# ChangUk/RecommenderSystems

Measured on AMD Instinct MI355X. Metric: RWR seeds/sec + achieved HBM GB/s on 100M-edge bipartite graph, 1/2/4/8 GPUs, higher is better.
Workload: dtype f64

## Files before the change

include/rwr.h:

```cpp
#ifndef RWR_H
#define RWR_H

#include <stdint.h>

#ifdef __cplusplus
extern "C" {
#endif

#define RWR_VERSION_STRING "0.4.0"

enum {
    RWR_OK            = 0,
    RWR_E_INVALID     = 1,
    RWR_E_RANGE       = 2,
    RWR_E_NO_DEVICE   = 3,
    RWR_E_HIP         = 4,
    RWR_E_NOMEM       = 5,
    RWR_E_CAPACITY    = 6,
    RWR_E_UNSUPPORTED = 7
};

enum { RWR_NODE_UNDEFINED = 0, RWR_NODE_USER = 1, RWR_NODE_ITEM = 2, RWR_NODE_ETC = 3 };
enum { RWR_EDGE_UNDEFINED = 0, RWR_EDGE_LIKE = 1, RWR_EDGE_FRIENDSHIP = 2, RWR_EDGE_FOLLOW = 3,
       RWR_EDGE_MENTION = 4, RWR_EDGE_AUTHORSHIP = 5, RWR_EDGE_PURCHASE = 6, RWR_EDGE_ETC = 7 };
// ... 17 lines not shown
} rwr_opts;

typedef struct rwr_stats {
    int32_t struct_size;
    int32_t n;
    int64_t nnz_raw;
    int64_t nnz;
    int32_t uniform;
    int32_t tile_seeds;
    int32_t tile_group;
    int32_t mode;
    double  build_ms;
    double  spmm_ms;
    int64_t spmm_launches;
    int64_t spmm_seed_steps;
    double  chain_ms;
    int64_t chain_launches;
    double  rank_ms;
    double  iterate_wall_ms;
    double  total_wall_ms;
    int64_t seeds_done;
    int64_t chain_redo_blocks;
    double  spmm_dense_ms;
    int64_t spmm_dense_launches;
    int64_t spmm_dense_seed_steps;
    int32_t uniform_path;
    int32_t reserved1;
    int64_t frontier_list_launches;
    int64_t rank_fused_groups;
    int64_t rank_fused_fallbacks;
    int64_t rank_pruned_rows;
    double  rank_bound_ms;
    int64_t x_clear_skipped;
} rwr_stats;


const char *rwr_version(void);
int32_t rwr_device_count(void);
const char *rwr_last_error(void);

int32_t rwr_graph_create(int32_t n, const int64_t *node_id, const uint8_t *node_type,
                         const int64_t *rowptr , const int32_t *dst, const uint8_t *etype,
                         const double *w, const rwr_opts *opts , rwr_graph **out);
int32_t rwr_graph_destroy(rwr_graph *g);
int32_t rwr_graph_update_links(rwr_graph *g, int64_t count, const int64_t *link_index,
                               const uint8_t *etype , const double *w );
int32_t rwr_graph_append_links(rwr_graph *g, int64_t count, const int32_t *src, const int32_t *dst,
                               const uint8_t *etype, const double *w,
                               int64_t *new_index_out );
int32_t rwr_graph_append_nodes(rwr_graph *g, int32_t n_new, const int64_t *node_id,
                               const uint8_t *node_type, int64_t count, const int32_t *src,
                               const int32_t *dst, const uint8_t *etype, const double *w,
                               int64_t *new_index_out );
int32_t rwr_graph_size(const rwr_graph *g, int32_t *n, int64_t *nnz_raw, int64_t *nnz_explicit);
int32_t rwr_graph_get_normalized(rwr_graph *g, double *w_out , uint8_t *dangling_out );

int32_t rwr_recommend(rwr_graph *g, int32_t seed, float d, int32_t n_iter, int32_t top_n,
                      int64_t *out_id, double *out_score, int64_t *inout_count);

int32_t rwr_recommend_eval(rwr_graph *g, int32_t seed, float d, int32_t n_iter, const int64_t *test_ids,
                           int64_t n_test, int64_t *n_hits, double *sum_precision, int64_t *list_len);

int32_t rwr_recommend_eval_batch(rwr_graph *g, const int32_t *seeds, int32_t K, float d, int32_t n_iter,
                                 const int64_t *test_ptr, const int64_t *test_ids, int64_t *n_hits,
                                 double *sum_precision, int64_t *list_len);

// ... 59 lines not shown
```

recommendersystems_amd/_lib.py:

```python
from __future__ import annotations

import ctypes as C
import os

_HERE = os.path.dirname(os.path.abspath(__file__))
LIB_PATH = os.path.join(_HERE, "librwr.so")

RWR_OK, RWR_E_INVALID, RWR_E_RANGE, RWR_E_NO_DEVICE, RWR_E_HIP, RWR_E_NOMEM, RWR_E_CAPACITY, RWR_E_UNSUPPORTED = range(8)
RWR_MODE_EXACT = 0
RWR_RUN_ITERATIONS, RWR_RUN_THRESHOLD, RWR_RUN_DEFAULT_THRESHOLD = 0, 1, 2

EXPORTS = [
    "rwr_version", "rwr_device_count", "rwr_last_error",
    "rwr_graph_create", "rwr_graph_update_links", "rwr_graph_append_links", "rwr_graph_append_nodes", "rwr_graph_destroy", "rwr_graph_size", "rwr_graph_get_normalized",
    "rwr_recommend", "rwr_recommend_eval", "rwr_recommend_eval_batch", "rwr_eval_graphs", "rwr_recommend_batch", "rwr_model_run", "rwr_model_deliver",
    "rwr_model_run_restart", "rwr_model_deliver_restart", "rwr_model_run_batch", "rwr_model_run_restart_batch",
    "rwr_recommend_restart_batch", "rwr_recommend_restart_eval_batch", "rwr_recommend_typed_batch",
    "rwr_part_begin", "rwr_part_step", "rwr_part_local_step", "rwr_part_finish_step", "rwr_part_rank",
    "rwr_get_stats", "rwr_reset_stats",
]


class rwr_opts(C.Structure):
    _fields_ = [("struct_size", C.c_int32), ("device", C.c_int32), ("mode", C.c_int32),
                ("tile_seeds", C.c_int32), ("tile_group", C.c_int32), ("profile", C.c_int32),
                ("workspace_bytes", C.c_int64), ("seed_row_kernel", C.c_int32), ("reserved0", C.c_int32)]


class rwr_graph_desc(C.Structure):
    _fields_ = [("n_nodes", C.c_int32), ("reserved0", C.c_int32), ("node_id", C.POINTER(C.c_int64)),
                ("node_type", C.POINTER(C.c_uint8)), ("rowptr", C.POINTER(C.c_int64)), ("dst", C.POINTER(C.c_int32)),
                ("etype", C.POINTER(C.c_uint8)), ("w", C.POINTER(C.c_double))]


class rwr_stats(C.Structure):
    _fields_ = [("struct_size", C.c_int32), ("n", C.c_int32), ("nnz_raw", C.c_int64), ("nnz", C.c_int64),
                ("uniform", C.c_int32), ("tile_seeds", C.c_int32), ("tile_group", C.c_int32), ("mode", C.c_int32),
                ("build_ms", C.c_double), ("spmm_ms", C.c_double), ("spmm_launches", C.c_int64),
                ("spmm_seed_steps", C.c_int64), ("chain_ms", C.c_double), ("chain_launches", C.c_int64),
                ("rank_ms", C.c_double), ("iterate_wall_ms", C.c_double), ("total_wall_ms", C.c_double),
                ("seeds_done", C.c_int64), ("chain_redo_blocks", C.c_int64),
                ("spmm_dense_ms", C.c_double), ("spmm_dense_launches", C.c_int64), ("spmm_dense_seed_steps", C.c_int64),
                ("uniform_path", C.c_int32), ("reserved1", C.c_int32), ("frontier_list_launches", C.c_int64),
                ("rank_fused_groups", C.c_int64), ("rank_fused_fallbacks", C.c_int64),
                ("rank_pruned_rows", C.c_int64), ("rank_bound_ms", C.c_double), ("x_clear_skipped", C.c_int64)]


class RwrError(RuntimeError):
    def __init__(self, status: int, message: str):
        super().__init__(f"librwr status {status}: {message}")
        self.status = status


_lib = None


def load():
    global _lib
    if _lib is not None:
        return _lib
    if not os.path.exists(LIB_PATH):
        raise ImportError(f"{LIB_PATH} not found: build it with `python -c 'import __graft_entry__ as g; g.build()'` "
                          "(hipcc --offload-arch=gfx950); there is no CPU fallback")
    lib = C.CDLL(LIB_PATH)
    p = C.POINTER
    lib.rwr_version.restype = C.c_char_p
    lib.rwr_last_error.restype = C.c_char_p
    lib.rwr_device_count.restype = C.c_int32
    lib.rwr_graph_create.restype = C.c_int32
    lib.rwr_graph_create.argtypes = [C.c_int32, p(C.c_int64), p(C.c_uint8), p(C.c_int64), p(C.c_int32),
                                     p(C.c_uint8), p(C.c_double), p(rwr_opts), p(C.c_void_p)]
    lib.rwr_graph_update_links.restype = C.c_int32
    lib.rwr_graph_update_links.argtypes = [C.c_void_p, C.c_int64, p(C.c_int64), p(C.c_uint8), p(C.c_double)]
    lib.rwr_graph_append_links.restype = C.c_int32
    lib.rwr_graph_append_links.argtypes = [C.c_void_p, C.c_int64, p(C.c_int32), p(C.c_int32), p(C.c_uint8), p(C.c_double),
                                           p(C.c_int64)]
    lib.rwr_graph_append_nodes.restype = C.c_int32
    lib.rwr_graph_append_nodes.argtypes = [C.c_void_p, C.c_int32, p(C.c_int64), p(C.c_uint8), C.c_int64, p(C.c_int32), p(C.c_int32),
# ... 72 lines not shown
```

recommendersystems_amd/csrc/api.hip:

```cpp
#include <stdarg.h>
#include <algorithm>
#include <cmath>
#include <vector>
#include <string.h>

#include "eval_plan.h"
#include "exclude_plan.h"
#include "handle.h"
#include "rank.h"

namespace rwr {

static thread_local char g_err[512] = "";

void set_error(const char *fmt, ...)
{
    va_list ap;
    va_start(ap, fmt);
    vsnprintf(g_err, sizeof(g_err), fmt, ap);
    va_end(ap);
}

template <class F>
static int32_t bound(const char *who, rwr_graph *g, F &&body)
// ... 602 lines not shown
}

int32_t rwr_part_rank(rwr_graph *g, void *dev_x, int32_t top_n, int64_t *ids, double *scores, int32_t *counts)
{
    g_err[0] = 0;
    if (!g || !dev_x || !ids || !scores || !counts) { set_error("rwr_part_rank: NULL argument"); return RWR_E_INVALID; }
    return bound("rwr_part_rank", g, [&] { return part_rank(g, (double *)dev_x, top_n, ids, scores, counts); });
}

int32_t rwr_get_stats(rwr_graph *g, rwr_stats *out)
{
    if (!g || !out) { set_error("rwr_get_stats: NULL argument"); return RWR_E_INVALID; }
    size_t sz = out->struct_size > 0 ? (size_t)out->struct_size : sizeof(rwr_stats);
    if (sz > sizeof(rwr_stats)) sz = sizeof(rwr_stats);
    rwr_stats s = g->stats;
    s.struct_size = (int32_t)sz;
    memcpy(out, &s, sz);
    return RWR_OK;
}

int32_t rwr_reset_stats(rwr_graph *g)
{
    if (!g) { set_error("rwr_reset_stats: NULL argument"); return RWR_E_INVALID; }
    rwr_stats &s = g->stats;
    s.spmm_ms = s.chain_ms = s.rank_ms = s.iterate_wall_ms = s.total_wall_ms = 0;
    s.spmm_launches = s.spmm_seed_steps = s.chain_launches = s.seeds_done = s.chain_redo_blocks = 0;
    s.spmm_dense_ms = 0;
    s.spmm_dense_launches = s.spmm_dense_seed_steps = 0;
    s.frontier_list_launches = 0;
    s.rank_fused_groups = s.rank_fused_fallbacks = 0;
    s.rank_pruned_rows = 0;
    s.rank_bound_ms = 0;
    s.x_clear_skipped = 0;
    return RWR_OK;
}

}
```

recommendersystems_amd/csrc/engine.h:

```cpp
#pragma once
#include <cstdlib>
#include <new>

#include "cand_plan.h"
#include "common.h"
#include "stage_layout.h"

struct rwr_graph {
    int32_t device = 0;
    int32_t n = 0;
    int64_t nnz_raw = 0;
    int64_t nnz = 0;
    int32_t n_items = 0;
    uint64_t id_key_top = 0;
    int32_t id_key_bits = 64;
    uint64_t id_key_lo = 0;
    int32_t id_key_lo_known = 0;
    int32_t uniform = 0;
    int32_t vf = 0;
    int32_t nonneg = 1;
    int32_t max_in_deg = 0;
    int32_t staged = 0;
    int32_t stage_pending = 0;
    int32_t poisoned = 0;
// ... 29 lines not shown
    rwr::DevBuf<int32_t> tail_rows[TAIL_MAX];
    int32_t tail_n[TAIL_MAX] = {0, 0, 0, 0};
    int32_t tail_depth = 0;
    std::vector<uint8_t> h_tail_flag;
    int32_t tail_state = 0;
    rwr::DevBuf<int32_t> cand_rows[rwr::CAND_CACHE];
    rwr::CandEntry cand_entry[rwr::CAND_CACHE];
    uint64_t cand_calls = 0;

    int32_t sw_state = 0, sw_B = 0, sw_BN = 0, sw_K = 0, sw_nwg = 0, sw_wpg = 0, sw_hub0 = 0;
    int32_t sw_rows = 0;
    int32_t sw_partial = 0;
    rwr::DevBuf<uint32_t> sw_wgblk;
    int64_t sw_words = 0;
    rwr::DevBuf<int32_t> sw_order;
    rwr::DevBuf<uint4> sw_meta;
    rwr::DevBuf<uint2> sw_ent;

    rwr::DevBuf<double> X, Y;
    rwr::DevBuf<int32_t> sm_tab;
    void *sm_pin = nullptr;
    void *sm_stage = nullptr;
    uint8_t *sm_out = nullptr;
    const uint8_t *stage_dev_ext = nullptr;
    rwr::DevBuf<uint8_t> d_stage;
    int32_t sm_pin_count = -1;
    rwr::DevBuf<double> Z0, Z1;
    rwr::DevBuf<int32_t> d_seeds;
    rwr::DevBuf<int32_t> d_slot_k;
    rwr::DevBuf<double> d_part;
    rwr::DevBuf<unsigned int> d_gate;
    rwr::DevBuf<uint32_t> d_nz;
    rwr::DevBuf<int32_t> fl_rows;
    rwr::DevBuf<int64_t> d_evoff;
    rwr::DevBuf<double> d_evterm;
    rwr::DevBuf<double> cs_approx;
    rwr::DevBuf<int32_t> cs_e;
    rwr::DevBuf<long long> cs_d0, cs_d1;
    rwr::DevBuf<double> cs_side;
    rwr::DevBuf<double> cs_mx;
    rwr::DevBuf<int32_t> cs_lnk;
    rwr::DevBuf<int32_t> cs_lnk0;
    rwr::DevBuf<double> cs_diff;
    rwr::DevBuf<double> cs_sums;
    rwr::DevBuf<int32_t> mb_row;
    rwr::DevBuf<unsigned long long> cs_redo;
    rwr::DevBuf<uint64_t> keys, keys_alt;
    rwr::DevBuf<uint32_t> vals, vals_alt;
    rwr::DevBuf<uint8_t> sort_temp;
    rwr::DevBuf<uint8_t> fused_ws;
    rwr::DevBuf<uint8_t> bound_ws;
    int32_t bound_first = -1, bound_lo = 0, bound_hi = 0;
    rwr::DevBuf<int64_t> d_out_id;
    rwr::DevBuf<double> d_out_score;
    rwr::DevBuf<int32_t> d_counts;

    int32_t part_lo = 0, part_hi = 0, part_G = 0, part_K = 0;
    int32_t part_steps = 0;
    double part_c1 = 0;
    std::vector<int32_t> part_seeds;

    hipStream_t stream = nullptr, stream2 = nullptr;
    hipStream_t stream3 = nullptr;
    hipEvent_t ev_h0 = nullptr, ev_h1 = nullptr;
    hipEvent_t ev_fork = nullptr, ev_join = nullptr;
    hipEvent_t ev_a = nullptr, ev_b = nullptr, ev_c = nullptr, ev_d = nullptr;
// ... 152 lines not shown
```

recommendersystems_amd/csrc/iterate.h:

```cpp
#pragma once
#include "column_ends.h"
#include "engine.h"
#include "rank.h"
#include "step_plan.h"

#include <new>
#include <optional>

namespace rwr {

struct RowScore {
    int32_t row, pad;
    double score;
};
struct SelSink {
    const double *tau = nullptr;
    int32_t *cursor = nullptr;
    RowScore *cand = nullptr;
    int32_t cap = 0, stride = 0;
    int32_t *overflow = nullptr;
    const int32_t *list = nullptr, *list_cnt = nullptr;
    int64_t list_stride = 0;
};

struct SpmmArgs {
    const double *X = nullptr;
    double *Y = nullptr;
    const int32_t *seeds = nullptr;
    double c1 = 0.0;
    bool skip_seed_row = false;
    const uint32_t *nz_in = nullptr;
    uint32_t *nz_out = nullptr;
    const uint32_t *act = nullptr;
    const double *Zin = nullptr;
    double *Zout = nullptr;
    bool hub_scan = false;
    RowSource rows{};
    int32_t row_first = 0, row_count = -1;
    const SelSink *sel = nullptr;
};
void launch_spmm(rwr_graph *g, int G, int tg, const SpmmArgs &a, hipStream_t s);
void launch_init_seeds(rwr_graph *g, int G, int tg, double *X, const int32_t *seeds, uint32_t *nz, double *Z, double c1,
                       hipStream_t s);
void launch_make_z(int64_t elems, int G, const double *X, double *Z, const double *w_src, double c1, hipStream_t s);
void launch_make_z_nz(rwr_graph *g, int32_t lo, int32_t hi, int G, const double *X, double *Zs, double c1, uint32_t *nz,
                      hipStream_t s);
void launch_mark_active(rwr_graph *g, int G, int tg, const uint32_t *nz, uint32_t *act, const int32_t *seeds, int32_t *fl_rows,
                        int32_t *fl_cnt, hipStream_t s);

struct Profile {
    const bool on;
    std::vector<hipEvent_t> pool, spmm, chain, rank, iter, bound;
    size_t used = 0;
    std::vector<uint8_t> dense;
    explicit Profile(const rwr_graph *g) : on(g->opts.profile != 0) {}
    ~Profile() { for (auto e : pool) (void)hipEventDestroy(e); }
    int32_t record(hipEvent_t &e, hipStream_t s);
    int32_t end(std::vector<hipEvent_t> &stage, hipEvent_t a, hipStream_t s);
    void reset() { spmm.clear(); chain.clear(); rank.clear(); iter.clear(); bound.clear(); dense.clear(); used = 0; }
    int32_t fold(rwr_graph *g);
};

struct GroupIter {
    rwr_graph *g;
    int G, tg;
    const int32_t *d_seeds;
    const int64_t *d_evoff;
    double c1;
    double *X, *Y;
    double *Zc = nullptr, *Zn = nullptr;
    uint32_t *nz_cur = nullptr, *nz_oth = nullptr;
    PlanConfig cfg;
// ... 68 lines not shown
```

recommendersystems_amd/csrc/iterate.hip:

```cpp
#include "iterate.h"
#include "spmm_chunk.h"

#include <climits>
#include <cstdlib>
#include <type_traits>

namespace rwr {

template <int G, bool VF>
__global__ __launch_bounds__(256) void k_spmm(int32_t n, const int64_t *__restrict__ in_ptr,
                                              const int32_t *__restrict__ in_src,
                                              const double *__restrict__ in_w,
                                              const int32_t *__restrict__ row_order, int32_t nrows,
                                              const double *__restrict__ X, double *__restrict__ Y,
                                              const int32_t *__restrict__ seeds, double c1, int skip_seed_row,
                                              const double *__restrict__ w_src, double *__restrict__ Zout)
{
    constexpr int RPW = WAVE / G;
    constexpr int U = 4;
    const int tile = blockIdx.y;
    const size_t toff = (size_t)tile * (size_t)n * G;
    X += toff;
    Y += toff;
    if (VF && Zout) Zout += toff;
// ... 16 lines not shown
            int32_t idx[U];
            double wv[U], xv[U];
#pragma unroll
            for (int u = 0; u < U; ++u) idx[u] = in_src[p + u];
#pragma unroll
            for (int u = 0; u < U; ++u) wv[u] = VF ? 0.0 : in_w[p + u];
#pragma unroll
            for (int u = 0; u < U; ++u) xv[u] = X[(size_t)idx[u] * G + k];
#pragma unroll
            for (int u = 0; u < U; ++u) {
                if (VF) {
                    acc += xv[u];
                } else {
                    double rw = c1 * xv[u];
                    acc += rw * wv[u];
                }
            }
        }
        for (; p < e; ++p) {
            if (VF) {
                acc += X[(size_t)in_src[p] * G + k];
            } else {
                double rw = c1 * X[(size_t)in_src[p] * G + k];
                acc += rw * in_w[p];
            }
        }
        if (j >= 0 && j != my_seed) {
            Y[(size_t)j * G + k] = acc;
            if (VF && Zout) { const double rw = c1 * acc; Zout[(size_t)j * G + k] = rw * w_src[j]; }
        }
    }
}

template <int G, int CH, bool CHECK, bool WRITE, bool VF, bool SEL = false>
__device__ __forceinline__ void spmm_chunked_body(int32_t n, const int64_t *__restrict__ in_ptr,
                                                  const int32_t *__restrict__ in_src,
                                                  const double *__restrict__ in_w,
                                                  const int32_t *__restrict__ row_order, int32_t nrows,
                                                  const double *__restrict__ X, double *__restrict__ Y,
                                                  const int32_t *__restrict__ seeds, double c1,
                                                  int skip_seed_row, const uint32_t *__restrict__ nz_in,
                                                  uint32_t *__restrict__ nz_out,
                                                  const uint32_t *__restrict__ act,
                                                  const double *__restrict__ w_src, double *__restrict__ Zout,
                                                  const SelSink sink = SelSink{})
{
    static_assert(G >= 8 && G <= 64, "chunked SpMM needs 8 <= G <= 64");
    static_assert(!SEL || (!CHECK && !WRITE), "the selecting form probes and writes no bitmap");
    constexpr int RPW = WAVE / G;
    constexpr int LW = G <= 32 ? G : VF ? 32 : CH;
    static_assert(LW % CH == 0 && CH <= LW, "an index load is a whole number of gather rounds");
    const int tile = blockIdx.y;
    const size_t toff = (size_t)tile * (size_t)n * G;
    X += toff;
    if (!SEL) Y += toff;
    if (VF && Zout) Zout += toff;
    const size_t nzw = ((size_t)n + 31) / 32;
    if (CHECK) nz_in += (size_t)tile * nzw;
    if (WRITE) nz_out += (size_t)tile * nzw;
    if (CHECK && act) act += (size_t)tile * nzw;
    const int lane = threadIdx.x & (WAVE - 1);
    const int sub = lane / G, k = lane % G;
    const int gbase = (lane - k) << 2;
    const int32_t my_seed = skip_seed_row ? seeds[tile * G + k] : -1;
    bool sel_real = false;
    double sel_tau = 0.0;
    if (SEL) {
        sel_real = seeds[tile * G + k] >= 0;
        sel_tau = sink.tau[tile * G + k];
    }
    const int wpb = blockDim.x / WAVE;
    const int64_t nwaves = (int64_t)gridDim.x * wpb;
    for (int64_t rb = ((int64_t)blockIdx.x * wpb + threadIdx.x / WAVE) * RPW; rb < nrows; rb += nwaves * RPW) {
        const int64_t r = rb + sub;
        int32_t j = -1;
        int64_t p = 0, e = 0;
        if (r < nrows) {
            j = row_order[r];
            p = in_ptr[j];
            e = in_ptr[j + 1];
            if (CHECK && act && !((act[(uint32_t)j >> 5] >> (j & 31)) & 1u)) e = p;
        }
        double acc = 0.0;
        while (__any(p < e)) {
            const int cnt = spmm_next_load(p, e - p, LW);
            int32_t my_idx = 0;
            double my_w = 0.0;
            if (k < cnt) {
                my_idx = in_src[p + k];
                if (!VF) my_w = in_w[p + k];
                if (CHECK) {
                    const uint32_t wd = nz_in[(uint32_t)my_idx >> 5];
                    if (!((wd >> (my_idx & 31)) & 1u)) my_idx |= (int32_t)0x80000000;
                }
            }
            const int wlo = __double2loint(my_w), whi = __double2hiint(my_w);
            unsigned long long um = 0;
            if (CHECK) {
                um = __ballot(k < cnt && my_idx >= 0);
                if (G < 64) {
#pragma unroll
                    for (int sh = G; sh < 64; sh <<= 1) um |= um >> sh;
                    um &= (1ull << (G & 63)) - 1ull;
                }
            }
#pragma unroll G == 64 ? LW / CH : 1
            for (int r0 = 0; r0 < LW; r0 += CH) {
                if (r0 > 0 && !__any(cnt > r0)) break;
                if (CHECK) {
                    unsigned long long rm = (um >> r0) & ((1ull << CH) - 1ull);
                    if (__popcll(rm) <= 4) {
                        while (rm) {
                            const int t = r0 + __builtin_ctzll(rm);
                            rm &= rm - 1;
                            const int idx = __builtin_amdgcn_ds_bpermute(gbase + (t << 2), my_idx);
                            if (VF) {
                                if (t < cnt && idx >= 0) acc += X[(size_t)idx * G + k];
                            } else {
                                const int lo = __builtin_amdgcn_ds_bpermute(gbase + (t << 2), wlo);
                                const int hi = __builtin_amdgcn_ds_bpermute(gbase + (t << 2), whi);
                                if (t < cnt && idx >= 0) {
                                    const double rw = c1 * X[(size_t)idx * G + k];
                                    acc += rw * __hiloint2double(hi, lo);
                                }
// ... 63 lines not shown
}

template <int G, int CH, bool VF>
__global__ __launch_bounds__(256) void k_spmm_select(int32_t n, const int64_t *__restrict__ in_ptr,
                                                     const int32_t *__restrict__ in_src,
                                                     const double *__restrict__ in_w,
                                                     const int32_t *__restrict__ rows, int32_t nrows,
                                                     const double *__restrict__ X, const int32_t *__restrict__ seeds,
                                                     double c1, const SelSink sink)
{
    if (sink.list) {
        rows = sink.list + (size_t)blockIdx.y * (size_t)sink.list_stride;
        nrows = sink.list_cnt[blockIdx.y];
    }
    spmm_chunked_body<G, CH, false, false, VF, true>(n, in_ptr, in_src, in_w, rows, nrows, X, nullptr, seeds, c1, 1, nullptr,
                                                     nullptr, nullptr, nullptr, nullptr, sink);
}

template <int G, int CH, bool VF>
__global__ __launch_bounds__(256) void k_spmm_frontier(int32_t n, const int64_t *__restrict__ in_ptr,
                                                       const int32_t *__restrict__ in_src,
                                                       const double *__restrict__ in_w,
                                                       const int32_t *__restrict__ fl_rows,
                                                       const int32_t *__restrict__ fl_cnt,
                                                       const double *__restrict__ X, double *__restrict__ Y,
                                                       const int32_t *__restrict__ seeds, double c1,
                                                       int skip_seed_row, const uint32_t *__restrict__ nz_in,
                                                       uint32_t *__restrict__ nz_out,
                                                       const double *__restrict__ w_src, double *__restrict__ Zout)
{
    const int tile = blockIdx.y;
    spmm_chunked_body<G, CH, true, true, VF>(n, in_ptr, in_src, in_w, fl_rows + (size_t)tile * (size_t)n, fl_cnt[tile], X, Y,
                                             seeds, c1, skip_seed_row, nz_in, nz_out, nullptr, w_src, Zout);
}

__global__ __launch_bounds__(256) void k_mark_active(int32_t n, const uint32_t *__restrict__ nz, uint32_t *__restrict__ act,
                                                     const int64_t *__restrict__ rowptr, const int32_t *__restrict__ dst,
                                                     const uint8_t *__restrict__ etype, int G, const int32_t *__restrict__ seeds,
                                                     int32_t *__restrict__ fl_rows, int32_t *__restrict__ fl_cnt)
{
    const size_t nzw = ((size_t)n + 31) / 32;
    const int tile = blockIdx.y;
    const int lane = threadIdx.x & (WAVE - 1);
    const size_t wi = (size_t)blockIdx.x * (blockDim.x / WAVE) + threadIdx.x / WAVE;
    uint32_t *a = act + (size_t)tile * nzw;
    int32_t *list = fl_rows ? fl_rows + (size_t)tile * (size_t)n : nullptr;
    if (list && blockIdx.x == 0 && threadIdx.x < (unsigned)G) {
        const int32_t sr = seeds[tile * G + threadIdx.x];
        if (sr >= 0) {
            const uint32_t bit = 1u << (sr & 31);
            if (!(atomicOr(&a[(uint32_t)sr >> 5], bit) & bit)) list[atomicAdd(&fl_cnt[tile], 1)] = sr;
        }
    }
    if (wi >= nzw) return;
    uint32_t w = nz[(size_t)tile * nzw + wi];
    while (w) {
        const int b = __builtin_ctz(w);
        w &= w - 1;
        const int64_t i = (int64_t)wi * 32 + b;
        const int64_t p1 = rowptr[i + 1];
        if (!list) {
            for (int64_t p = rowptr[i] + lane; p < p1; p += WAVE)
                if (etype[p] != RWR_EDGE_UNDEFINED) {
                    const int32_t t = dst[p];
                    atomicOr(&a[(uint32_t)t >> 5], 1u << (t & 31));
                }
// ... 376 lines not shown
    if (j >= lo && j < hi) {
        const double w = w_src[j];
        const size_t at = (size_t)(j - lo) * G;
        for (int k = 0; k < G; ++k) {
            const double xv = X[(size_t)j * G + k];
            const double rw = c1 * xv;
            Zs[at + k] = rw * w;
            any = any || xv != 0.0;
        }
    }
    const unsigned long long m = __ballot(any);
    const int lane = threadIdx.x & (WAVE - 1);
    if (lane == 0 && (uint32_t)m) nz[(uint64_t)j >> 5] = (uint32_t)m;
    if (lane == 32 && (uint32_t)(m >> 32)) nz[(uint64_t)j >> 5] = (uint32_t)(m >> 32);
}


static PlanInput read_plan_knobs()
{
    PlanInput v;
    const char *e;
    if ((e = getenv("RWR_SPMM"))) v.spmm = atoi(e);
    if ((e = RWR_TUNE_ENV("RWR_NZ_ITERS"))) v.nz_iters = atoi(e);
    if ((e = getenv("RWR_ACT_ITERS"))) v.act_iters = atoi(e);
    if ((e = RWR_TUNE_ENV("RWR_ACT_MIN_N"))) v.act_min_n = atol(e);
    if ((e = getenv("RWR_FRONTIER_LIST"))) v.frontier_list = atoi(e);
    if ((e = getenv("RWR_CHAIN"))) v.chain = atoi(e);
    if ((e = RWR_TUNE_ENV("RWR_SCAN_WORK"))) v.scan_work = atof(e);
    if ((e = RWR_TUNE_ENV("RWR_SCAN_SIDE"))) v.scan_side = atoi(e);
    if ((e = RWR_TUNE_ENV("RWR_GATE"))) v.gate = atoi(e);
    if ((e = getenv("RWR_TAIL_ROWS"))) v.tail_rows = atoi(e);
    if ((e = RWR_TUNE_ENV("RWR_CHAIN_SERIAL"))) v.two_streams = atoi(e) == 0;
    if ((e = getenv("RWR_X_CLEAR"))) v.x_clear = atoi(e);
    return v;
}
static const PlanInput &plan_knobs() { static const PlanInput k = read_plan_knobs(); return k; }

template <class F> static void bool_dispatch(F &&f) { f(); }
template <class F, class... B> static void bool_dispatch(F &&f, bool b, B... bs)
{
    bool_dispatch([&](auto... c) { if (b) f(std::true_type{}, c...); else f(std::false_type{}, c...); }, bs...);
}

template <int G>
static void launch_spmm_g(rwr_graph *g, int tg, const SpmmArgs &a, hipStream_t s)
{
    const bool vf = a.Zin != nullptr;
    const double *GS = vf ? a.Zin : a.X;
    const int skip = a.skip_seed_row;
    constexpr int RPW = WAVE / G;
    constexpr int CH = G > 16 ? 16 : G;
    if constexpr (G >= 8) {
        if (a.rows.kind == Rows::Frontier) {
            const int32_t *fl_rows = g->fl_rows.p, *fl_cnt = g->fl_rows.p + (size_t)tg * (size_t)g->n;
            const unsigned want = cdiv((size_t)g->n / 10 + 1, (size_t)RPW * 4);
            const unsigned gx = want < 1u ? 1u : want < 2048u ? want : 2048u;
            bool_dispatch([&](auto v) {
                hipLaunchKernelGGL((k_spmm_frontier<G, CH, decltype(v)::value>), dim3(gx, tg), dim3(256), 0, s, g->n, g->in_ptr.p,
                                   g->in_src.p, g->in_w.p, fl_rows, fl_cnt, GS, a.Y, a.seeds, a.c1, skip, a.nz_in, a.nz_out,
                                   g->w_src.p, a.Zout);
            }, vf);
            return;
        }
    }
    const bool listed = a.rows.kind == Rows::Tail;
    const int32_t *order = listed ? g->tail_rows[a.rows.level].p : g->row_order.p;
    int32_t nrows = listed ? g->tail_n[a.rows.level] : g->n;
    if (listed) {
        const int32_t first = a.row_first < nrows ? a.row_first : nrows;
        order += first;
        nrows = (a.row_count >= 0 && a.row_count < nrows - first) ? a.row_count : nrows - first;
    }
    if (nrows <= 0 && (a.sel || a.row_count >= 0)) return;
    unsigned want = cdiv((size_t)nrows, (size_t)RPW * 4);
    unsigned gx = want < 1u ? 1u : want < 8192u ? want : 8192u;
    if constexpr (G == 1) {
        if (tg == 1 && plan_knobs().spmm != 0) {
            launch_spmv_exact(g, a.X, a.Y, a.seeds, a.c1, skip, a.act, a.nz_out, s, a.Zin, a.Zout, a.hub_scan);
            return;
        }
    }
    if constexpr (G >= 8) {
        if (a.sel) {
            const SelSink sink = *a.sel;
            bool_dispatch([&](auto v) {
                hipLaunchKernelGGL((k_spmm_select<G, CH, decltype(v)::value>), dim3(gx, tg), dim3(256), 0, s, g->n, g->in_ptr.p,
                                   g->in_src.p, g->in_w.p, order, nrows, GS, a.seeds, a.c1, sink);
            }, vf);
            return;
        }
    }
    if constexpr (G >= 8) {
        if (plan_knobs().spmm != 0) {
            bool_dispatch([&](auto chk, auto wr, auto v, auto lst) {
                if constexpr (decltype(chk)::value || !decltype(wr)::value)
                    hipLaunchKernelGGL((k_spmm_chunked<G, CH, decltype(chk)::value, decltype(wr)::value, decltype(v)::value,
                                                       decltype(lst)::value>), dim3(gx, tg), dim3(256), 0, s, g->n, g->in_ptr.p,
                                       g->in_src.p, g->in_w.p, order, nrows, GS, a.Y, a.seeds, a.c1, skip, a.nz_in, a.nz_out,
                                       a.act, g->w_src.p, a.Zout);
            }, a.nz_in != nullptr, a.nz_in && a.nz_out, vf, listed);
            return;
        }
    }
    bool_dispatch([&](auto v) {
        hipLaunchKernelGGL((k_spmm<G, decltype(v)::value>), dim3(gx, tg), dim3(256), 0, s, g->n, g->in_ptr.p, g->in_src.p,
                           g->in_w.p, order, nrows, GS, a.Y, a.seeds, a.c1, skip, g->w_src.p, a.Zout);
    }, vf);
}
void launch_spmm(rwr_graph *g, int G, int tg, const SpmmArgs &a, hipStream_t s)
{
    RWR_DISPATCH_G(G, launch_spmm_g<GG>(g, tg, a, s));
}
void launch_init_seeds(rwr_graph *g, int G, int tg, double *X, const int32_t *seeds, uint32_t *nz, double *Z, double c1,
                       hipStream_t s)
{
    hipLaunchKernelGGL(k_init_seeds, dim3(cdiv((size_t)tg * G, 64)), dim3(64), 0, s, g->n, tg, G, X, seeds, nz, Z, g->w_src.p, c1);
}
void launch_make_z(int64_t elems, int G, const double *X, double *Z, const double *w_src, double c1, hipStream_t s)
{
    hipLaunchKernelGGL(k_make_z, dim3(cdiv((size_t)elems, 256)), dim3(256), 0, s, elems, G, X, Z, w_src, c1);
}
void launch_make_z_nz(rwr_graph *g, int32_t lo, int32_t hi, int G, const double *X, double *Zs, double c1, uint32_t *nz,
                      hipStream_t s)
{
    const int64_t first = (int64_t)lo & ~(int64_t)63;
// ... 67 lines not shown
            *acc += ms;
        }
        return RWR_OK;
    };
    if (on) {
        RWR_TRY(drain(spmm, &g->stats.spmm_dense_ms, true));
        RWR_TRY(drain(spmm, &g->stats.spmm_ms, false));
        RWR_TRY(drain(chain, &g->stats.chain_ms, false));
        RWR_TRY(drain(rank, &g->stats.rank_ms, false));
        RWR_TRY(drain(iter, &g->stats.iterate_wall_ms, false));
        RWR_TRY(drain(bound, &g->stats.rank_bound_ms, false));
    }
    reset();
    return RWR_OK;
}

int32_t GroupIter::init(bool fresh, bool ranks_nonneg, bool ranking_only)
{
    const int32_t n = g->n;
    hipStream_t s = g->stream;
    const size_t elems = (size_t)tg * (size_t)n * G;
    PlanInput in = plan_knobs();
    in.n = n; in.nnz = g->nnz; in.nonneg = g->nonneg; in.big_n = spmv_big_n(); in.seed_row_kernel = g->opts.seed_row_kernel;
    in.scan_self = chain_scan_self_contained(G); in.G = G; in.tg = tg; in.c1 = c1;
    in.fresh = fresh; in.ranks_nonneg = ranks_nonneg; in.ranking_only = ranking_only;
    cfg = plan_config(in);
    if (!fresh && Zc) launch_make_z((int64_t)elems, G, X, Zc, g->w_src.p, c1, s);
    const size_t nzw = ((size_t)n + 31) / 32;
    if (cfg.flist && g->fl_rows.ensure((size_t)tg * (size_t)n + (size_t)tg) != RWR_OK) {
        (void)hipGetLastError();
        cfg.flist = false;
        cfg.clear_x = plan_clear_x(cfg);
    }
    if (fresh && cfg.clear_x) RWR_HIP(hipMemsetAsync(X, 0, elems * sizeof(double), s));
    if (fresh && !cfg.clear_x) g->stats.x_clear_skipped += 1;
    if (fresh && Zc && !cfg.flist) RWR_HIP(hipMemsetAsync(Zc, 0, elems * sizeof(double), s));
    nz_cur = cfg.nz_iters > 0 ? g->d_nz.p : nullptr;
    nz_oth = cfg.nz_iters > 0 ? g->d_nz.p + (size_t)tg * nzw : nullptr;
    if (nz_cur) RWR_HIP(hipMemsetAsync(nz_cur, 0, (size_t)tg * nzw * sizeof(uint32_t), s));
    if (fresh) launch_init_seeds(g, G, tg, X, d_seeds, nz_cur, Zc, c1, s);
    RWR_HIP(hipGetLastError());
    if (cfg.scan) RWR_TRY(chain_scan_prepare(g, G, tg, d_seeds, s));
    if (Zc && G == 1 && tg == 1 && cfg.addends_nonneg) RWR_TRY(sweep_prepare(g));
    if (Zc && cfg.chain_kind == 0 && !cfg.scan) RWR_TRY(ensure_in_w(g));
    return RWR_OK;
}

int32_t GroupIter::step(const StepPlan &p, Profile &prof, int32_t row_first, int32_t row_count)
{
    const int32_t n = g->n;
    hipStream_t s = g->stream;
    const size_t nzw = ((size_t)n + 31) / 32;
    constexpr int GATE_SLOTS = 64;
    const uint32_t *nz_in = p.probe ? nz_cur : nullptr;
    uint32_t *nz_out = p.write_bits ? nz_oth : nullptr;
    if (nz_out) RWR_HIP(hipMemsetAsync(nz_out, 0, (size_t)tg * nzw * sizeof(uint32_t), s));
    uint32_t *act = p.mark ? g->d_nz.p + 2 * (size_t)tg * nzw : nullptr;
    const bool listed = p.rows.kind == Rows::Frontier;
    if (act) {
        int32_t *fl_rows = listed ? g->fl_rows.p : nullptr, *fl_cnt = listed ? fl_rows + (size_t)tg * (size_t)n : nullptr;
        RWR_HIP(hipMemsetAsync(act, 0, (size_t)tg * nzw * sizeof(uint32_t), s));
        if (fl_cnt) RWR_HIP(hipMemsetAsync(fl_cnt, 0, (size_t)tg * sizeof(int32_t), s));
        launch_mark_active(g, G, tg, nz_in, act, d_seeds, fl_rows, fl_cnt, s);
    }
    const uint32_t *nz_terms = p.terms_nz ? nz_in : nullptr;
    double *zout = (Zc && p.form_z) ? Zn : nullptr;
    hipStream_t sc = p.chain_side ? g->stream2 : s;
    unsigned int *gate_it = p.gate ? g->d_gate.p + (it % GATE_SLOTS) : nullptr;
    if (p.chain != Chain::None) {
        if (!p.scan()) RWR_DISPATCH_G(G, launch_seed_terms<GG>(g, tg, X, d_seeds, c1, d_evoff, s, Zc, nz_terms));
        if (gate_it) RWR_HIP(hipMemsetAsync(gate_it, 0, sizeof(unsigned int), s));
        if (p.chain_side) { RWR_HIP(hipEventRecord(g->ev_fork, s)); RWR_HIP(hipStreamWaitEvent(sc, g->ev_fork, 0)); }
        if (p.scan() && !(p.chain_self && Zc)) RWR_DISPATCH_G(G, launch_seed_terms<GG>(g, tg, X, d_seeds, c1, d_evoff, sc, Zc, nz_terms));
        hipEvent_t c0; RWR_TRY(prof.record(c0, sc));
        if (p.scan())
            RWR_TRY(chain_scan_step(g, G, tg, X, Y, d_seeds, d_evoff, c1, nz_out, sc, p.chain_self ? Zc : nullptr,
                                    p.chain_self ? zout : nullptr));
        else
            RWR_DISPATCH_G(G, launch_chain<GG>(g, tg, X, Y, d_seeds, c1, d_evoff, nz_out, gate_it, sc, p.chain, nz_in,
                                                       p.chain_masked));
        RWR_TRY(prof.end(prof.chain, c0, sc));
        if (p.chain_side) RWR_HIP(hipEventRecord(g->ev_join, sc));
    }
    if (gate_it) hipLaunchKernelGGL(k_gate, dim3(1), dim3(1), 0, s, gate_it, (unsigned)(tg < 192 ? tg : 192));
    hipEvent_t a; RWR_TRY(prof.record(a, s));
    SpmmArgs sp;
    sp.X = X, sp.Y = Y, sp.seeds = d_seeds, sp.c1 = c1, sp.skip_seed_row = true;
    sp.nz_in = nz_in, sp.nz_out = nz_out, sp.act = act, sp.Zin = Zc, sp.Zout = zout;
    sp.hub_scan = cfg.addends_nonneg, sp.rows = p.rows;
    sp.row_first = row_first, sp.row_count = row_count;
    launch_spmm(g, G, tg, sp, s);
    RWR_TRY(prof.end(prof.spmm, a, s));
    if (prof.on) prof.dense.push_back(p.dense());
    if (p.dense()) { g->stats.spmm_dense_launches += 1; ++dense_steps; }
    if (p.chain_side) RWR_HIP(hipStreamWaitEvent(s, g->ev_join, 0));
    if (zout && p.seed_z) hipLaunchKernelGGL(k_seed_z, dim3(cdiv((size_t)tg * G, 64)), dim3(64), 0, s, n, tg, G, Y, zout, d_seeds, g->w_src.p, c1);
    RWR_HIP(hipGetLastError());
    { double *t = X; X = Y; Y = t; }
    { double *t = Zc; Zc = Zn; Zn = t; }
    { uint32_t *tz = nz_cur; nz_cur = nz_oth; nz_oth = tz; }
    g->stats.spmm_launches += 1;
    g->stats.chain_launches += p.chain != Chain::None; g->stats.frontier_list_launches += listed;
    ++it;
    return RWR_OK;
}

int32_t GroupIter::redo_rows(const StepPlan &p, Profile &prof, int32_t row_first, int32_t row_count, const SelSink *sel)
{
    hipStream_t s = g->stream;
    hipEvent_t a; RWR_TRY(prof.record(a, s));
    SpmmArgs sp;
    sp.X = Y, sp.Y = X, sp.seeds = d_seeds, sp.c1 = c1, sp.skip_seed_row = true;
    sp.Zin = Zn, sp.Zout = nullptr;
    sp.hub_scan = cfg.addends_nonneg, sp.rows = p.rows;
    sp.row_first = row_first, sp.row_count = row_count, sp.sel = sel;
    launch_spmm(g, G, tg, sp, s);
    RWR_TRY(prof.end(prof.spmm, a, s));
    if (prof.on) prof.dense.push_back(0);
    RWR_HIP(hipGetLastError());
    return RWR_OK;
}

int32_t iterate_group(rwr_graph *g, int G, int tg, const int32_t *d_seeds, const int64_t *d_evoff, const int32_t *h_seeds,
// ... 30 lines not shown
```

recommendersystems_amd/csrc/step_plan.h:

```cpp
#pragma once

#include <cstdint>

namespace rwr {

struct PlanInput {
    int spmm = 1, nz_iters = 4, act_iters = -1, frontier_list = 1, chain = 1, x_clear = 0;
    int64_t act_min_n = 200000; double scan_work = 10000.0;
    int scan_side = 1, gate = 1, tail_rows = 1;
    bool two_streams = true;
    int32_t n = 0, big_n = 2000000;
    int64_t nnz = 0; bool nonneg = true;
    int seed_row_kernel = 0;
    bool scan_self = false;
    int G = 1, tg = 1;
    double c1 = 0.85;
    bool fresh = true;
    bool ranks_nonneg = true;
    bool ranking_only = false;
};

struct PlanConfig {
    int G = 1, tg = 1; bool fresh = true;
    int nz_iters = 0;
    int act_iters = 0;
    bool flist = false;
    bool addends_nonneg = false;
    bool scan = false;
    int chain_kind = 1;
    bool scan_side = false, scan_self = false;
    bool two_streams = true, gate = true;
    bool tails = false; int tail_depth = 0;
    unsigned need = 0;
    bool force_clear = false;
    bool clear_x = true;
};

inline bool plan_clear_x(const PlanConfig &c) { return c.force_clear || !c.flist || c.scan || c.chain_kind == 0; }

inline PlanConfig plan_config(const PlanInput &in)
{
    PlanConfig c;
    c.G = in.G, c.tg = in.tg, c.fresh = in.fresh;
    const bool single = in.G == 1 && in.tg == 1;
    c.nz_iters = (in.G >= 8 && in.spmm != 0 && in.nonneg) ? in.nz_iters : 0;
    c.act_iters = in.act_iters >= 0 ? in.act_iters : ((in.nnz / (in.n > 0 ? in.n : 1)) <= 64 ? 2 : 1);
    if (single && in.act_iters < 0 && c.act_iters == 2 && in.n >= in.big_n) c.act_iters = 3;
    if (single && in.spmm != 0 && in.nonneg) c.nz_iters = c.act_iters;
    if (single && in.act_iters < 0 && in.n < in.act_min_n) c.nz_iters = c.act_iters = 0;
    if (!in.fresh) c.nz_iters = c.act_iters = 0;
    c.flist = in.ranking_only && in.fresh && in.frontier_list != 0 && in.G >= 8 && c.nz_iters >= 2 && c.act_iters >= 1;
    c.chain_kind = in.seed_row_kernel == 1 ? 3 : in.seed_row_kernel == 2 ? 2 : in.seed_row_kernel == 3 ? 0 : in.chain;
    const double per_seed = 0.89 * (double)in.nnz / (double)(in.n > 0 ? in.n : 1) + 6.7;
    c.addends_nonneg = in.c1 >= 0.0 && in.c1 <= 1.0 && in.nonneg && in.ranks_nonneg;
    c.scan = c.addends_nonneg && (c.chain_kind == 2 || (c.chain_kind == 1 && (double)in.tg * in.G * per_seed < in.scan_work));
    c.scan_side = in.scan_side != 0 && single && in.two_streams && in.n >= 100000;
    c.scan_self = in.scan_self, c.two_streams = in.two_streams, c.gate = in.gate != 0;
    c.tails = in.ranking_only && in.tail_rows != 0 && !single;
    c.force_clear = in.x_clear != 0;
    c.clear_x = plan_clear_x(c);
    return c;
}

enum class Rows : uint8_t { All, Frontier, Tail };
struct RowSource { Rows kind = Rows::All; int level = 0; };
enum class Chain : uint8_t { None, Scan, ScanSide, Sparse, Roles, Simple };

struct StepPlan {
    RowSource rows;
    bool probe = false, write_bits = false;
    bool mark = false;
    bool terms_nz = false;
    Chain chain = Chain::None;
    bool chain_masked = false;
    bool chain_side = false, gate = false;
    bool chain_self = false;
    bool form_z = false, seed_z = false;
    bool dense() const { return !probe && rows.kind == Rows::All; }
    bool scan() const { return chain == Chain::Scan || chain == Chain::ScanSide; }
};

inline int last_tail(const PlanConfig &c)
{
    for (int k = 0; c.tails && k < c.tail_depth; ++k)
        if ((c.need >> k) & 1u) return k;
    return c.tails ? c.tail_depth - 1 : -1;
}

inline bool step_lists(const PlanConfig &c, int64_t it, int64_t T)
{
    const int64_t k = T - 1 - it;
    if (!c.flist || T < 0 || it < 0 || k <= 0 || k <= last_tail(c)) return false;
    const bool write_bits = it + 1 < c.nz_iters, mark = it < c.nz_iters && it < c.act_iters;
    return mark && write_bits && (it + 1 < c.act_iters || it == 1);
}

inline StepPlan plan_step(const PlanConfig &c, int64_t it, int64_t T)
{
    StepPlan p;
    const int64_t k = T - 1 - it;
    const bool last = T >= 0 && k == 0, tail = T >= 0 && k <= last_tail(c);
    p.probe = it < c.nz_iters;
    p.write_bits = it + 1 < c.nz_iters;
    p.mark = p.probe && it < c.act_iters;
    p.terms_nz = c.flist && p.probe;
    if (tail)
        p.rows = {Rows::Tail, (int)k};
    else if (step_lists(c, it, T))
        p.rows = {Rows::Frontier, 0};
    if (tail && !((c.need >> k) & 1u)) p.chain = Chain::None;
    else if (c.scan && (!p.mark || c.G == 1)) p.chain = c.scan_side ? Chain::ScanSide : Chain::Scan;
    else if (p.mark) p.chain = Chain::Sparse;
    else p.chain = c.chain_kind == 0 ? Chain::Simple : Chain::Roles;
    p.chain_masked = !c.clear_x && p.chain != Chain::None && p.chain != Chain::Sparse && step_lists(c, it - 1, T);
    const bool fold = p.chain != Chain::None && !p.scan();
    p.chain_side = p.chain == Chain::ScanSide || (fold && c.two_streams);
    p.gate = fold && c.two_streams && c.gate;
    p.chain_self = p.scan() && c.scan_self;
    p.form_z = !last;
    p.seed_z = p.form_z && p.chain != Chain::None && !p.chain_self;
    return p;
}

}
```

Measured before the change: 859.3.

## Precompute per-edge liveness masks to replace random bitmap probes in SpMM

Adds an entry-live path. Each probing step transposes the per-tile nonzero bitmaps into per-node 32-tile words, then expands them into one mask word per CSR entry. The SpMM kernel then reads that mask word instead of gathering a bitmap word indexed by the source node. The goal is to turn scattered bitmap reads into a streamed read aligned with the edge arrays, at the cost of two extra kernels per step that touch every edge and up to several GB of extra workspace. The path is enabled by default only for graphs with at least 100M edges in ranking-only fresh runs.

```diff
diff --git a/include/rwr.h b/include/rwr.h
--- a/include/rwr.h
+++ b/include/rwr.h
@@ -73,6 +73,7 @@
     int64_t rank_pruned_rows;
     double  rank_bound_ms;
     int64_t x_clear_skipped;
+    int64_t entry_live_launches;
 } rwr_stats;
 
 
diff --git a/recommendersystems_amd/_lib.py b/recommendersystems_amd/_lib.py
--- a/recommendersystems_amd/_lib.py
+++ b/recommendersystems_amd/_lib.py
@@ -43,7 +43,8 @@
                 ("spmm_dense_ms", C.c_double), ("spmm_dense_launches", C.c_int64), ("spmm_dense_seed_steps", C.c_int64),
                 ("uniform_path", C.c_int32), ("reserved1", C.c_int32), ("frontier_list_launches", C.c_int64),
                 ("rank_fused_groups", C.c_int64), ("rank_fused_fallbacks", C.c_int64),
-                ("rank_pruned_rows", C.c_int64), ("rank_bound_ms", C.c_double), ("x_clear_skipped", C.c_int64)]
+                ("rank_pruned_rows", C.c_int64), ("rank_bound_ms", C.c_double), ("x_clear_skipped", C.c_int64),
+                ("entry_live_launches", C.c_int64)]
 
 
 class RwrError(RuntimeError):
diff --git a/recommendersystems_amd/csrc/api.hip b/recommendersystems_amd/csrc/api.hip
--- a/recommendersystems_amd/csrc/api.hip
+++ b/recommendersystems_amd/csrc/api.hip
@@ -658,7 +658,8 @@
     s.rank_pruned_rows = 0;
     s.rank_bound_ms = 0;
     s.x_clear_skipped = 0;
-    return RWR_OK;
-}
-
-}
+    s.entry_live_launches = 0;
+    return RWR_OK;
+}
+
+}
diff --git a/recommendersystems_amd/csrc/engine.h b/recommendersystems_amd/csrc/engine.h
--- a/recommendersystems_amd/csrc/engine.h
+++ b/recommendersystems_amd/csrc/engine.h
@@ -85,6 +85,7 @@
     rwr::DevBuf<unsigned int> d_gate;
     rwr::DevBuf<uint32_t> d_nz;
     rwr::DevBuf<int32_t> fl_rows;
+    rwr::DevBuf<uint32_t> ent_nzT, ent_live;
     rwr::DevBuf<int64_t> d_evoff;
     rwr::DevBuf<double> d_evterm;
     rwr::DevBuf<double> cs_approx;
diff --git a/recommendersystems_amd/csrc/iterate.h b/recommendersystems_amd/csrc/iterate.h
--- a/recommendersystems_amd/csrc/iterate.h
+++ b/recommendersystems_amd/csrc/iterate.h
@@ -38,6 +38,7 @@
     RowSource rows{};
     int32_t row_first = 0, row_count = -1;
     const SelSink *sel = nullptr;
+    const uint32_t *ent_live = nullptr;
 };
 void launch_spmm(rwr_graph *g, int G, int tg, const SpmmArgs &a, hipStream_t s);
 void launch_init_seeds(rwr_graph *g, int G, int tg, double *X, const int32_t *seeds, uint32_t *nz, double *Z, double c1,
diff --git a/recommendersystems_amd/csrc/iterate.hip b/recommendersystems_amd/csrc/iterate.hip
--- a/recommendersystems_amd/csrc/iterate.hip
+++ b/recommendersystems_amd/csrc/iterate.hip
@@ -72,7 +72,7 @@
     }
 }
 
-template <int G, int CH, bool CHECK, bool WRITE, bool VF, bool SEL = false>
+template <int G, int CH, bool CHECK, bool WRITE, bool VF, bool SEL = false, bool LIVE = false>
 __device__ __forceinline__ void spmm_chunked_body(int32_t n, const int64_t *__restrict__ in_ptr,
                                                   const int32_t *__restrict__ in_src,
                                                   const double *__restrict__ in_w,
@@ -83,10 +83,12 @@
                                                   uint32_t *__restrict__ nz_out,
                                                   const uint32_t *__restrict__ act,
                                                   const double *__restrict__ w_src, double *__restrict__ Zout,
-                                                  const SelSink sink = SelSink{})
+                                                  const SelSink sink = SelSink{},
+                                                  const uint32_t *__restrict__ ent_live = nullptr)
 {
     static_assert(G >= 8 && G <= 64, "chunked SpMM needs 8 <= G <= 64");
     static_assert(!SEL || (!CHECK && !WRITE), "the selecting form probes and writes no bitmap");
+    static_assert(!LIVE || CHECK, "the per-link masks replace the bitmap probe");
     constexpr int RPW = WAVE / G;
     constexpr int LW = G <= 32 ? G : VF ? 32 : CH;
     static_assert(LW % CH == 0 && CH <= LW, "an index load is a whole number of gather rounds");
@@ -96,7 +98,7 @@
     if (!SEL) Y += toff;
     if (VF && Zout) Zout += toff;
     const size_t nzw = ((size_t)n + 31) / 32;
-    if (CHECK) nz_in += (size_t)tile * nzw;
+    if (CHECK && !LIVE) nz_in += (size_t)tile * nzw;
     if (WRITE) nz_out += (size_t)tile * nzw;
     if (CHECK && act) act += (size_t)tile * nzw;
     const int lane = threadIdx.x & (WAVE - 1);
@@ -129,7 +131,9 @@
             if (k < cnt) {
                 my_idx = in_src[p + k];
                 if (!VF) my_w = in_w[p + k];
-                if (CHECK) {
+                if (LIVE) {
+                    if (!((ent_live[p + k] >> (tile & 31)) & 1u)) my_idx |= (int32_t)0x80000000;
+                } else if (CHECK) {
                     const uint32_t wd = nz_in[(uint32_t)my_idx >> 5];
                     if (!((wd >> (my_idx & 31)) & 1u)) my_idx |= (int32_t)0x80000000;
                 }
@@ -259,6 +263,56 @@
     const int tile = blockIdx.y;
     spmm_chunked_body<G, CH, true, true, VF>(n, in_ptr, in_src, in_w, fl_rows + (size_t)tile * (size_t)n, fl_cnt[tile], X, Y,
                                              seeds, c1, skip_seed_row, nz_in, nz_out, nullptr, w_src, Zout);
+}
+
+__global__ __launch_bounds__(256) void k_nz_transpose(int32_t n, int tg, const uint32_t *__restrict__ nz, uint32_t *__restrict__ nzT)
+{
+    const int64_t i = (int64_t)blockIdx.x * blockDim.x + threadIdx.x;
+    if (i >= n) return;
+    const size_t nzw = ((size_t)n + 31) / 32;
+    const int slab = blockIdx.y;
+    uint32_t out = 0;
+#pragma unroll 8
+    for (int t = 0; t < 32; ++t) {
+        const int tile = slab * 32 + t;
+        if (tile < tg) out |= ((nz[(size_t)tile * nzw + (size_t)(i >> 5)] >> (i & 31)) & 1u) << t;
+    }
+    nzT[(size_t)slab * (size_t)n + (size_t)i] = out;
+}
+__global__ __launch_bounds__(256) void k_entry_live(int64_t nnz, int32_t n, int slabs, const int32_t *__restrict__ in_src,
+                                                    const uint32_t *__restrict__ nzT, uint32_t *__restrict__ live)
+{
+    constexpr int U = 4;
+    const int64_t stride = (int64_t)gridDim.x * blockDim.x;
+    for (int64_t e0 = (int64_t)blockIdx.x * blockDim.x + threadIdx.x; e0 < nnz; e0 += U * stride) {
+        int32_t src[U];
+#pragma unroll
+        for (int u = 0; u < U; ++u) src[u] = e0 + u * stride < nnz ? in_src[e0 + u * stride] : -1;
+        for (int sl = 0; sl < slabs; ++sl) {
+            uint32_t v[U];
+#pragma unroll
+            for (int u = 0; u < U; ++u) v[u] = src[u] >= 0 ? nzT[(size_t)sl * (size_t)n + (size_t)src[u]] : 0u;
+#pragma unroll
+            for (int u = 0; u < U; ++u)
+                if (src[u] >= 0) live[(size_t)sl * (size_t)nnz + (size_t)(e0 + u * stride)] = v[u];
+        }
+    }
+}
+template <int G, int CH, bool WRITE, bool VF>
+__global__ __launch_bounds__(256) void k_spmm_entry_live(int32_t n, const int64_t *__restrict__ in_ptr,
+                                                         const int32_t *__restrict__ in_src,
+                                                         const double *__restrict__ in_w,
+                                                         const int32_t *__restrict__ row_order, int32_t nrows,
+                                                         const double *__restrict__ X, double *__restrict__ Y,
+                                                         const int32_t *__restrict__ seeds, double c1,
+                                                         int skip_seed_row, uint32_t *__restrict__ nz_out,
+                                                         const uint32_t *__restrict__ act,
+                                                         const double *__restrict__ w_src, double *__restrict__ Zout,
+                                                         const uint32_t *__restrict__ live, int64_t nnz)
+{
+    spmm_chunked_body<G, CH, true, WRITE, VF, false, true>(n, in_ptr, in_src, in_w, row_order, nrows, X, Y, seeds, c1,
+                                                           skip_seed_row, nullptr, nz_out, act, w_src, Zout, SelSink{},
+                                                           live + (size_t)(blockIdx.y >> 5) * (size_t)nnz);
 }
 
 __global__ __launch_bounds__(256) void k_mark_active(int32_t n, const uint32_t *__restrict__ nz, uint32_t *__restrict__ act,
@@ -701,9 +755,19 @@
     if ((e = getenv("RWR_TAIL_ROWS"))) v.tail_rows = atoi(e);
     if ((e = RWR_TUNE_ENV("RWR_CHAIN_SERIAL"))) v.two_streams = atoi(e) == 0;
     if ((e = getenv("RWR_X_CLEAR"))) v.x_clear = atoi(e);
+    if ((e = getenv("RWR_ENTRY_LIVE"))) v.entry_live = atoi(e);
     return v;
 }
 static const PlanInput &plan_knobs() { static const PlanInput k = read_plan_knobs(); return k; }
+static size_t entry_live_cap_bytes()
+{
+    static const size_t v = [] {
+        const char *e = getenv("RWR_ENTRY_LIVE_CAP_MB");
+        const long long mb = e ? atoll(e) : 4096;
+        return (size_t)(mb > 0 ? mb : 0) << 20;
+    }();
+    return v;
+}
 
 template <class F> static void bool_dispatch(F &&f) { f(); }
 template <class F, class... B> static void bool_dispatch(F &&f, bool b, B... bs)
@@ -760,6 +824,16 @@
         }
     }
     if constexpr (G >= 8) {
+        if (a.ent_live && a.nz_in && !listed && plan_knobs().spmm != 0) {
+            bool_dispatch([&](auto wr, auto v) {
+                hipLaunchKernelGGL((k_spmm_entry_live<G, CH, decltype(wr)::value, decltype(v)::value>), dim3(gx, tg), dim3(256), 0,
+                                   s, g->n, g->in_ptr.p, g->in_src.p, g->in_w.p, order, nrows, GS, a.Y, a.seeds, a.c1, skip,
+                                   a.nz_out, a.act, g->w_src.p, a.Zout, a.ent_live, g->nnz);
+            }, a.nz_out != nullptr, vf);
+            return;
+        }
+    }
+    if constexpr (G >= 8) {
         if (plan_knobs().spmm != 0) {
             bool_dispatch([&](auto chk, auto wr, auto v, auto lst) {
                 if constexpr (decltype(chk)::value || !decltype(wr)::value)
@@ -893,6 +967,14 @@
         cfg.flist = false;
         cfg.clear_x = plan_clear_x(cfg);
     }
+    if (cfg.entry_live) {
+        const size_t slabs = ((size_t)tg + 31) / 32, words = slabs * (size_t)g->nnz;
+        if (g->nnz <= 0 || words > entry_live_cap_bytes() / sizeof(uint32_t) || g->ent_nzT.ensure(slabs * (size_t)n) != RWR_OK ||
+            g->ent_live.ensure(words) != RWR_OK) {
+            (void)hipGetLastError();
+            cfg.entry_live = false;
+        }
+    }
     if (fresh && cfg.clear_x) RWR_HIP(hipMemsetAsync(X, 0, elems * sizeof(double), s));
     if (fresh && !cfg.clear_x) g->stats.x_clear_skipped += 1;
     if (fresh && Zc && !cfg.flist) RWR_HIP(hipMemsetAsync(Zc, 0, elems * sizeof(double), s));
@@ -923,6 +1005,16 @@
         RWR_HIP(hipMemsetAsync(act, 0, (size_t)tg * nzw * sizeof(uint32_t), s));
         if (fl_cnt) RWR_HIP(hipMemsetAsync(fl_cnt, 0, (size_t)tg * sizeof(int32_t), s));
         launch_mark_active(g, G, tg, nz_in, act, d_seeds, fl_rows, fl_cnt, s);
+    }
+    const uint32_t *ent_live = nullptr;
+    if (p.entry_live && nz_in) {
+        const int slabs = (tg + 31) / 32;
+        hipLaunchKernelGGL(k_nz_transpose, dim3(cdiv((size_t)n, 256), slabs), dim3(256), 0, s, n, tg, nz_in, g->ent_nzT.p);
+        const unsigned want = cdiv((size_t)g->nnz, 256 * 4);
+        hipLaunchKernelGGL(k_entry_live, dim3(want < 1u ? 1u : want < (1u << 20) ? want : (1u << 20)), dim3(256), 0, s, g->nnz, n,
+                           slabs, g->in_src.p, g->ent_nzT.p, g->ent_live.p);
+        ent_live = g->ent_live.p;
+        g->stats.entry_live_launches += 1;
     }
     const uint32_t *nz_terms = p.terms_nz ? nz_in : nullptr;
     double *zout = (Zc && p.form_z) ? Zn : nullptr;
@@ -950,6 +1042,7 @@
     sp.nz_in = nz_in, sp.nz_out = nz_out, sp.act = act, sp.Zin = Zc, sp.Zout = zout;
     sp.hub_scan = cfg.addends_nonneg, sp.rows = p.rows;
     sp.row_first = row_first, sp.row_count = row_count;
+    sp.ent_live = ent_live;
     launch_spmm(g, G, tg, sp, s);
     RWR_TRY(prof.end(prof.spmm, a, s));
     if (prof.on) prof.dense.push_back(p.dense());
diff --git a/recommendersystems_amd/csrc/step_plan.h b/recommendersystems_amd/csrc/step_plan.h
--- a/recommendersystems_amd/csrc/step_plan.h
+++ b/recommendersystems_amd/csrc/step_plan.h
@@ -3,6 +3,8 @@
 #include <cstdint>
 
 namespace rwr {
+
+constexpr int64_t ENTRY_LIVE_MIN_NNZ = 100000000;
 
 struct PlanInput {
     int spmm = 1, nz_iters = 4, act_iters = -1, frontier_list = 1, chain = 1, x_clear = 0;
@@ -18,6 +20,8 @@
     bool fresh = true;
     bool ranks_nonneg = true;
     bool ranking_only = false;
+    int entry_live = 1;
+    int64_t entry_live_min_nnz = ENTRY_LIVE_MIN_NNZ;
 };
 
 struct PlanConfig {
@@ -34,9 +38,16 @@
     unsigned need = 0;
     bool force_clear = false;
     bool clear_x = true;
+    bool entry_live = false;
 };
 
 inline bool plan_clear_x(const PlanConfig &c) { return c.force_clear || !c.flist || c.scan || c.chain_kind == 0; }
+
+inline bool plan_entry_live(const PlanInput &in, const PlanConfig &c)
+{
+    if (in.entry_live == 0 || !in.ranking_only || !in.fresh || in.G < 8 || c.nz_iters <= 0) return false;
+    return in.entry_live == 2 || in.nnz >= in.entry_live_min_nnz;
+}
 
 inline PlanConfig plan_config(const PlanInput &in)
 {
@@ -59,6 +70,7 @@
     c.tails = in.ranking_only && in.tail_rows != 0 && !single;
     c.force_clear = in.x_clear != 0;
     c.clear_x = plan_clear_x(c);
+    c.entry_live = plan_entry_live(in, c);
     return c;
 }
 
@@ -76,6 +88,7 @@
     bool chain_side = false, gate = false;
     bool chain_self = false;
     bool form_z = false, seed_z = false;
+    bool entry_live = false;
     bool dense() const { return !probe && rows.kind == Rows::All; }
     bool scan() const { return chain == Chain::Scan || chain == Chain::ScanSide; }
 };
@@ -119,6 +132,7 @@
     p.chain_self = p.scan() && c.scan_self;
     p.form_z = !last;
     p.seed_z = p.form_z && p.chain != Chain::None && !p.chain_self;
+    p.entry_live = c.entry_live && c.G >= 8 && p.probe && p.rows.kind == Rows::All;
     return p;
 }
 
```

Result: faster. 875.8 (median of 6 runs) (+1.9%).
